# facebookresearch/pytorchvideo

Hardware: AMD Instinct MI355X
Metric: clips/sec forward (higher is better)
Workload: dtype bf16; 1 GPU; x3d_m: create_x3d(input_clip_length=16,input_crop_size=224) [B,3,16,224,224]; per_gpu_batch=32, global_batch=32, parallelism=dp1 (batch-sharded, logits all_gather), head_collective=none (one rank: the logits stay where they are), hip_graph=True, streams=2

## Files before the change

pytorchvideo_amd/csrc/pv_pwdw.hip:

```cpp
#include "pv_common.h"

int pv_plane_variant(const pv_dwconv3d_desc& d);
int pv_plane_tiles(const pv_dwconv3d_desc& d, int nw);

namespace {

constexpr int kPlaneThreads = 256;
constexpr int kPR = kPlaneThreads / 64;

template <int S, int NW, int KS, int ACT>
__global__ __launch_bounds__(kPlaneThreads) void pwdw_plane_kernel(const pv_dwconv3d_desc d, int ntiles, int ngroups) {
  constexpr int TW = 4 * NW;
  constexpr int IH = (kPR - 1) * S + 3;
  constexpr int IW = (TW - 1) * S + 3;
  constexpr bool kDeep = S == 1;
  constexpr int IWP = (IW + 1) & ~1;
  constexpr int NVOX = IH * IW;
  constexpr int NMT = (NVOX + 15) / 16;
  constexpr int MT = (NMT + kPR - 1) / kPR;
  constexpr int NC = (NW - 1) * S + 3;
  __shared__ __attribute__((aligned(16))) bf16_t s_in[2][IH * IWP + 1][32];
  __shared__ float s_ps[kPR][32];

  const int tid = threadIdx.x;
  const int lane = tid & 63;
  const int row = __builtin_amdgcn_readfirstlane(tid >> 6);
  const int cp = lane & 15;
  const int sx = lane >> 4;
  const int n16 = lane & 15, q = lane >> 4;
  const int c_p = pv_round_up(d.C, 8);
  const int xcd = blockIdx.x & 7, slot = blockIdx.x >> 3;
  const int grp = slot % ngroups;
  const long tb = (long)(slot / ngroups) * 8 + xcd;
  if (tb >= (long)ntiles * d.B) return;
  const int tile_id = (int)(tb % ntiles);
  const int cbase = grp * 32;
  const int ch = cbase + cp * 2;
  const bool ch_ok = ch < c_p;
  const int tiles_w = (d.Wo + TW - 1) / TW;
  const int th = tile_id / tiles_w, tw = tile_id - th * tiles_w;
  const int b = (int)(tb / ntiles);
  const int ho0 = th * kPR, wo0 = tw * TW;
  const int ho = ho0 + row, wo_first = wo0 + sx * NW;
  const int hi0 = ho0 * S - 1, wi0 = wo0 * S - 1;

  constexpr unsigned kOOB = 0x80000000u;
  const bf16_t* X = static_cast<const bf16_t*>(d.x) + (long)b * d.x_bs;
  bf16_t* Y = static_cast<bf16_t*>(d.y) + (long)b * d.y_bs;
  const unsigned x_plane_bytes = (unsigned)(d.Hi * d.Wi * d.ldx) * 2u;
  const unsigned y_plane_bytes = (unsigned)(d.Ho * d.Wo * d.ldy) * 2u;
  __amdgpu_buffer_rsrc_t rx = __builtin_amdgcn_make_buffer_rsrc((void*)X, 0, (int)(x_plane_bytes * (unsigned)d.Ti), 0x00020000);
  __amdgpu_buffer_rsrc_t ry = __builtin_amdgcn_make_buffer_rsrc((void*)Y, 0, (int)(y_plane_bytes * (unsigned)d.To), 0x00020000);

  float2 wt[27];
#pragma unroll
  for (int t = 0; t < 27; ++t)
    wt[t] = ch_ok ? *reinterpret_cast<const float2*>(d.w + (long)t * c_p + ch) : float2{0.f, 0.f};
  float2 sc = {0.f, 0.f}, sh = {0.f, 0.f};
  if (ch_ok) {
    sc.x = ch < d.C ? (d.scale ? d.scale[ch] : 1.f) : 0.f;
    sc.y = ch + 1 < d.C ? (d.scale ? d.scale[ch + 1] : 1.f) : 0.f;
    sh.x = ch < d.C ? (d.shift ? d.shift[ch] : 0.f) : 0.f;
    sh.y = ch + 1 < d.C ? (d.shift ? d.shift[ch + 1] : 0.f) : 0.f;
  }

  bf16x8 wa[2][KS];
  {
    const bf16_t* __restrict__ Wa = static_cast<const bf16_t*>(d.pw_w);
#pragma unroll
    for (int nt = 0; nt < 2; ++nt)
#pragma unroll
      for (int ks = 0; ks < KS; ++ks)
        wa[nt][ks] = *reinterpret_cast<const bf16x8*>(Wa + (long)(cbase + 8 * (n16 >> 2) + 4 * nt + (n16 & 3)) * (KS * 32) + ks * 32 + q * 8);
  }
  float2 sa[2][2], ha[2][2];
#pragma unroll
  for (int nt = 0; nt < 2; ++nt)
#pragma unroll
    for (int r = 0; r < 4; ++r) {
      const int c = cbase + q * 8 + nt * 4 + r;
      const bool ok = c < d.C;
      const float s_ = ok ? (d.pw_scale ? d.pw_scale[c] : 1.f) : 0.f;
      const float h_ = ok ? (d.pw_shift ? d.pw_shift[c] : 0.f) : 0.f;
      if (r & 1) { sa[nt][r >> 1].y = s_; ha[nt][r >> 1].y = h_; }
      else { sa[nt][r >> 1].x = s_; ha[nt][r >> 1].x = h_; }
    }
  const bool a_relu = d.pw_act == PV_ACT_RELU;

  auto colperm = [](int c) { return c ^ ((c / (NW * S)) & 1); };
  unsigned x_off[MT];
  int h_lds[MT];
#pragma unroll
  for (int i = 0; i < MT; ++i) {
    const int v = (row + i * kPR) * 16 + n16;
    const int ih = v / IW, iw = v - ih * IW;
    const int hi = hi0 + ih, wi = wi0 + iw;
    const bool in_tile = v < NVOX;
    const bool ok = in_tile && (unsigned)hi < (unsigned)d.Hi && (unsigned)wi < (unsigned)d.Wi;
    x_off[i] = ok ? (unsigned)((hi * d.Wi + wi) * d.ldx + q * 8) * 2u : kOOB;
    h_lds[i] = (in_tile ? ih * IWP + colperm(iw) : IH * IWP) * 32 + q * 8;
  }
  typedef unsigned int u32x4 __attribute__((ext_vector_type(4)));
  u32x4 xa[MT][KS], xb[MT][KS];
  auto load_plane = [&](u32x4 (&reg)[MT][KS], int p) {
    if (p >= d.Ti) return;
    const unsigned pb = (unsigned)p * x_plane_bytes;
#pragma unroll
    for (int i = 0; i < MT; ++i)
#pragma unroll
      for (int ks = 0; ks < KS; ++ks)
        reg[i][ks] = __builtin_amdgcn_raw_buffer_load_b128(rx, (int)(x_off[i] + pb + ks * 64u), 0, 0);
  };
  auto produce_plane = [&](const u32x4 (&reg)[MT][KS], int p) {
    if (p >= d.Ti) return;
    bf16_t* dst = &s_in[p & 1][0][0];
#pragma unroll
    for (int i = 0; i < MT; ++i) {
      f32x4 acc[2] = {f32x4{0.f, 0.f, 0.f, 0.f}, f32x4{0.f, 0.f, 0.f, 0.f}};
#pragma unroll
      for (int ks = 0; ks < KS; ++ks) {
        const bf16x8 xf = __builtin_bit_cast(bf16x8, reg[i][ks]);
        acc[0] = __builtin_amdgcn_mfma_f32_16x16x32_bf16(wa[0][ks], xf, acc[0], 0, 0, 0);
        acc[1] = __builtin_amdgcn_mfma_f32_16x16x32_bf16(wa[1][ks], xf, acc[1], 0, 0, 0);
      }
      const unsigned inside = x_off[i] != kOOB ? 0xffffffffu : 0u;
      u32x4 o;
#pragma unroll
      for (int nt = 0; nt < 2; ++nt) {
        typedef __bf16 bf16x2_t __attribute__((ext_vector_type(2)));
        typedef short s16x2 __attribute__((ext_vector_type(2)));
#pragma unroll
        for (int h = 0; h < 2; ++h) {
          const float v0 = acc[nt][2 * h] * sa[nt][h].x + ha[nt][h].x;
          const float v1 = acc[nt][2 * h + 1] * sa[nt][h].y + ha[nt][h].y;
          const bf16x2_t pk = {(bf16_t)v0, (bf16_t)v1};
          s16x2 pi = __builtin_bit_cast(s16x2, pk);
          if (a_relu) pi = __builtin_elementwise_max(pi, s16x2{0, 0});
          o[nt * 2 + h] = __builtin_bit_cast(unsigned, pi) & inside;
        }
      }
      *reinterpret_cast<u32x4*>(dst + h_lds[i]) = o;
    }
  };

  float2 acc[3][NW];
#pragma unroll
  for (int a = 0; a < 3; ++a)
#pragma unroll
    for (int n = 0; n < NW; ++n) acc[a][n] = float2{0.f, 0.f};
  float2 ps = {0.f, 0.f};

  unsigned y_off[NW];
  float y_mask[NW];
#pragma unroll
  for (int n = 0; n < NW; ++n) {
    const int wo = wo_first + n;
    const bool ok = ch_ok && ho < d.Ho && wo < d.Wo;
    y_off[n] = ok ? (unsigned)((ho * d.Wo + wo) * d.ldy + ch) * 2u : kOOB;
    y_mask[n] = ok ? 1.f : 0.f;
  }
  const bool has_psum = d.psum != nullptr;
  auto finalize = [&](float2 (&a)[NW], int t) {
    const unsigned tbytes = (unsigned)t * y_plane_bytes;
#pragma unroll
    for (int n = 0; n < NW; ++n) {
      float v0 = a[n].x * sc.x + sh.x, v1 = a[n].y * sc.y + sh.y;
      if (has_psum) { ps.x += v0 * y_mask[n]; ps.y += v1 * y_mask[n]; }
      if (ACT == PV_ACT_RELU) { v0 = fmaxf(v0, 0.f); v1 = fmaxf(v1, 0.f); }
      else if (ACT == PV_ACT_SWISH) { v0 *= pv_sigmoid(v0); v1 *= pv_sigmoid(v1); }
      typedef __bf16 bf16x2_t __attribute__((ext_vector_type(2)));
      const bf16x2_t o = {(bf16_t)v0, (bf16_t)v1};
      __builtin_amdgcn_raw_buffer_store_b32(__builtin_bit_cast(unsigned, o), ry, (int)(y_off[n] + tbytes), 0, 0);
    }
  };

  auto plane = [&](int p) {
    const bf16_t* base = &s_in[p & 1][0][0] + cp * 2;
#pragma unroll
    for (int dh = 0; dh < 3; ++dh) {
      float2 x[NC];
#pragma unroll
      for (int i = 0; i < NC; ++i) {
        const uint32_t u = *reinterpret_cast<const uint32_t*>(base + ((row * S + dh) * IWP + colperm(sx * NW * S + i)) * 32);
        x[i].x = __uint_as_float(u << 16);
        x[i].y = __uint_as_float(u & 0xffff0000u);
      }
#pragma unroll
      for (int dw = 0; dw < 3; ++dw) {
        const float2 w0 = wt[(0 * 3 + dh) * 3 + dw];
        const float2 w1 = wt[(1 * 3 + dh) * 3 + dw];
        const float2 w2 = wt[(2 * 3 + dh) * 3 + dw];
#pragma unroll
        for (int n = 0; n < NW; ++n) {
          const float2 xv = x[n * S + dw];
          acc[2][n].x += xv.x * w0.x; acc[2][n].y += xv.y * w0.y;
          acc[1][n].x += xv.x * w1.x; acc[1][n].y += xv.y * w1.y;
          acc[0][n].x += xv.x * w2.x; acc[0][n].y += xv.y * w2.y;
        }
      }
    }
    if (p >= 1) finalize(acc[0], p - 1);
    if (p == d.Ti - 1) finalize(acc[1], p);
#pragma unroll
    for (int n = 0; n < NW; ++n) {
      acc[0][n] = acc[1][n];
      acc[1][n] = acc[2][n];
      acc[2][n] = float2{0.f, 0.f};
    }
  };

  load_plane(xa, 0);
  if (kDeep) load_plane(xb, 1);
  produce_plane(xa, 0);
  __syncthreads();
  if (kDeep) {
    for (int p = 0; p < d.Ti; p += 2) {
      load_plane(xa, p + 2);
      plane(p);
      produce_plane(xb, p + 1);
      __syncthreads();
      if (p + 1 < d.Ti) {
        load_plane(xb, p + 3);
        plane(p + 1);
        produce_plane(xa, p + 2);
        __syncthreads();
      }
    }
  } else {
    for (int p = 0; p < d.Ti; ++p) {
      load_plane(xa, p + 1);
      plane(p);
      produce_plane(xa, p + 1);
      __syncthreads();
    }
  }

  if (d.psum != nullptr) {
    ps.x += __shfl_xor(ps.x, 16, 64); ps.y += __shfl_xor(ps.y, 16, 64);
    ps.x += __shfl_xor(ps.x, 32, 64); ps.y += __shfl_xor(ps.y, 32, 64);
    if (lane < 16) { s_ps[row][cp * 2] = ps.x; s_ps[row][cp * 2 + 1] = ps.y; }
    __syncthreads();
    if (tid < 32 && cbase + tid < c_p) {
      float a = 0.f;
#pragma unroll
      for (int rr = 0; rr < kPR; ++rr) a += s_ps[rr][tid];
      float* dst = d.psum + ((long)b * ntiles + tile_id) * c_p + cbase + tid;
      *dst = a;
    }
  }
}

template <int S, int NW, int KS> int launch_pwdw(const pv_dwconv3d_desc& d, hipStream_t s) {
  const int c_p = pv_round_up(d.C, 8);
  const int ntiles = pv_plane_tiles(d, NW), ngroups = (c_p + 31) / 32;
  const long blocks = pv_ceil_div((long)ntiles * d.B, 8) * 8 * ngroups;
  if (blocks > 0x7fffffffL) return PV_ERR_UNSUPPORTED;
  dim3 grid((unsigned)blocks), block(kPlaneThreads);
  if (d.act == PV_ACT_NONE) PV_LAUNCH((pwdw_plane_kernel<S, NW, KS, PV_ACT_NONE>), grid, block, 0, s, d, ntiles, ngroups);
  else if (d.act == PV_ACT_RELU) PV_LAUNCH((pwdw_plane_kernel<S, NW, KS, PV_ACT_RELU>), grid, block, 0, s, d, ntiles, ngroups);
  else PV_LAUNCH((pwdw_plane_kernel<S, NW, KS, PV_ACT_SWISH>), grid, block, 0, s, d, ntiles, ngroups);
  PV_LAUNCH_CHECK();
  return PV_OK;
}

template <int KS> int launch_ks(const pv_dwconv3d_desc& d, int nw, hipStream_t s) {
  if (d.sw == 1) return nw == 4 ? launch_pwdw<1, 4, KS>(d, s) : launch_pwdw<1, 2, KS>(d, s);
  return nw == 4 ? launch_pwdw<2, 4, KS>(d, s) : launch_pwdw<2, 2, KS>(d, s);
}

int ksteps_of(const pv_dwconv3d_desc& d) {
  const int ks = (d.pw_cin + 31) / 32;
  return (ks == 1 || ks == 2 || ks == 3 || ks == 4 || ks == 6) ? ks : 0;
}

}

int pv_pwdw_supported(const pv_dwconv3d_desc& d) {
  if (d.dtype != PV_BF16 || d.w_mod != 0 || d.n_prefix != 0) return 0;
  if (d.pw_cin <= 0 || d.ldx < pv_round_up(d.pw_cin, 8)) return 0;
  if (!ksteps_of(d)) return 0;
  if (d.pw_act != PV_ACT_NONE && d.pw_act != PV_ACT_RELU) return 0;
  return pv_plane_variant(d) != 0;
}

int pv_pwdw_launch(const pv_dwconv3d_desc& d, hipStream_t s) {
  if (!pv_pwdw_supported(d)) return PV_ERR_UNSUPPORTED;
  const int nw = pv_plane_variant(d);
  switch (ksteps_of(d)) {
    case 1: return launch_ks<1>(d, nw, s);
    case 2: return launch_ks<2>(d, nw, s);
    case 3: return launch_ks<3>(d, nw, s);
    case 4: return launch_ks<4>(d, nw, s);
    case 6: return launch_ks<6>(d, nw, s);
  }
  return PV_ERR_UNSUPPORTED;
}
```

Before: 11900 clips/s.

## Specialize pwdw plane kernel on relu/psum and software-pipeline pointwise MFMA epilogue

```diff
diff --git a/pytorchvideo_amd/csrc/pv_pwdw.hip b/pytorchvideo_amd/csrc/pv_pwdw.hip
--- a/pytorchvideo_amd/csrc/pv_pwdw.hip
+++ b/pytorchvideo_amd/csrc/pv_pwdw.hip
@@ -1,3 +1,5 @@
+#include <type_traits>
+
 #include "pv_common.h"
 
 int pv_plane_variant(const pv_dwconv3d_desc& d);
@@ -7,6 +9,19 @@
 
 constexpr int kPlaneThreads = 256;
 constexpr int kPR = kPlaneThreads / 64;
+
+__device__ __forceinline__ void mfma_first(f32x4& dst, const bf16x8& a, const bf16x8& b) {
+  asm volatile("v_mfma_f32_16x16x32_bf16 %0, %1, %2, 0" : "=&v"(dst) : "v"(a), "v"(b));
+}
+__device__ __forceinline__ void mfma_acc(f32x4& dst, const bf16x8& a, const bf16x8& b) {
+  asm volatile("v_mfma_f32_16x16x32_bf16 %0, %1, %2, %0" : "+v"(dst) : "v"(a), "v"(b));
+}
+__device__ __forceinline__ void mfma_wait(f32x4& c0, f32x4& c1) {
+  asm volatile("s_nop 7" : "+v"(c0), "+v"(c1));
+}
+template <typename V> __device__ __forceinline__ void mfma_after(f32x4& c0, f32x4& c1, const V& done) {
+  asm volatile("" : "+v"(c0), "+v"(c1) : "v"(done));
+}
 
 template <int S, int NW, int KS, int ACT>
 __global__ __launch_bounds__(kPlaneThreads) void pwdw_plane_kernel(const pv_dwconv3d_desc d, int ntiles, int ngroups) {
@@ -19,6 +34,8 @@
   constexpr int NMT = (NVOX + 15) / 16;
   constexpr int MT = (NMT + kPR - 1) / kPR;
   constexpr int NC = (NW - 1) * S + 3;
+  constexpr bool kTailStore = S == 1;
+  constexpr bool kArithMfma = KS <= 2;
   __shared__ __attribute__((aligned(16))) bf16_t s_in[2][IH * IWP + 1][32];
   __shared__ float s_ps[kPR][32];
 
@@ -52,10 +69,10 @@
   __amdgpu_buffer_rsrc_t rx = __builtin_amdgcn_make_buffer_rsrc((void*)X, 0, (int)(x_plane_bytes * (unsigned)d.Ti), 0x00020000);
   __amdgpu_buffer_rsrc_t ry = __builtin_amdgcn_make_buffer_rsrc((void*)Y, 0, (int)(y_plane_bytes * (unsigned)d.To), 0x00020000);
 
-  float2 wt[27];
+  f32x2 wt[27];
 #pragma unroll
   for (int t = 0; t < 27; ++t)
-    wt[t] = ch_ok ? *reinterpret_cast<const float2*>(d.w + (long)t * c_p + ch) : float2{0.f, 0.f};
+    wt[t] = ch_ok ? *reinterpret_cast<const f32x2*>(d.w + (long)t * c_p + ch) : f32x2{0.f, 0.f};
   float2 sc = {0.f, 0.f}, sh = {0.f, 0.f};
   if (ch_ok) {
     sc.x = ch < d.C ? (d.scale ? d.scale[ch] : 1.f) : 0.f;
@@ -85,9 +102,8 @@
       if (r & 1) { sa[nt][r >> 1].y = s_; ha[nt][r >> 1].y = h_; }
       else { sa[nt][r >> 1].x = s_; ha[nt][r >> 1].x = h_; }
     }
-  const bool a_relu = d.pw_act == PV_ACT_RELU;
-
   auto colperm = [](int c) { return c ^ ((c / (NW * S)) & 1); };
+  typedef unsigned int u32x4 __attribute__((ext_vector_type(4)));
   unsigned x_off[MT];
   int h_lds[MT];
 #pragma unroll
@@ -98,9 +114,13 @@
     const bool in_tile = v < NVOX;
     const bool ok = in_tile && (unsigned)hi < (unsigned)d.Hi && (unsigned)wi < (unsigned)d.Wi;
     x_off[i] = ok ? (unsigned)((hi * d.Wi + wi) * d.ldx + q * 8) * 2u : kOOB;
-    h_lds[i] = (in_tile ? ih * IWP + colperm(iw) : IH * IWP) * 32 + q * 8;
-  }
-  typedef unsigned int u32x4 __attribute__((ext_vector_type(4)));
+    h_lds[i] = (ok ? ih * IWP + colperm(iw) : IH * IWP) * 32 + q * 8;
+    if (in_tile && !ok) {
+      const int z = (ih * IWP + colperm(iw)) * 32 + q * 8;
+      *reinterpret_cast<u32x4*>(&s_in[0][0][0] + z) = u32x4{0u, 0u, 0u, 0u};
+      *reinterpret_cast<u32x4*>(&s_in[1][0][0] + z) = u32x4{0u, 0u, 0u, 0u};
+    }
+  }
   u32x4 xa[MT][KS], xb[MT][KS];
   auto load_plane = [&](u32x4 (&reg)[MT][KS], int p) {
     if (p >= d.Ti) return;
@@ -109,46 +129,30 @@
     for (int i = 0; i < MT; ++i)
 #pragma unroll
       for (int ks = 0; ks < KS; ++ks)
-        reg[i][ks] = __builtin_amdgcn_raw_buffer_load_b128(rx, (int)(x_off[i] + pb + ks * 64u), 0, 0);
+        reg[i][ks] = __builtin_amdgcn_raw_buffer_load_b128(rx, (int)(x_off[i] + ks * 64u), (int)pb, 0);
   };
-  auto produce_plane = [&](const u32x4 (&reg)[MT][KS], int p) {
-    if (p >= d.Ti) return;
-    bf16_t* dst = &s_in[p & 1][0][0];
-#pragma unroll
-    for (int i = 0; i < MT; ++i) {
-      f32x4 acc[2] = {f32x4{0.f, 0.f, 0.f, 0.f}, f32x4{0.f, 0.f, 0.f, 0.f}};
-#pragma unroll
-      for (int ks = 0; ks < KS; ++ks) {
-        const bf16x8 xf = __builtin_bit_cast(bf16x8, reg[i][ks]);
-        acc[0] = __builtin_amdgcn_mfma_f32_16x16x32_bf16(wa[0][ks], xf, acc[0], 0, 0, 0);
-        acc[1] = __builtin_amdgcn_mfma_f32_16x16x32_bf16(wa[1][ks], xf, acc[1], 0, 0, 0);
-      }
-      const unsigned inside = x_off[i] != kOOB ? 0xffffffffu : 0u;
-      u32x4 o;
-#pragma unroll
-      for (int nt = 0; nt < 2; ++nt) {
-        typedef __bf16 bf16x2_t __attribute__((ext_vector_type(2)));
-        typedef short s16x2 __attribute__((ext_vector_type(2)));
-#pragma unroll
-        for (int h = 0; h < 2; ++h) {
-          const float v0 = acc[nt][2 * h] * sa[nt][h].x + ha[nt][h].x;
-          const float v1 = acc[nt][2 * h + 1] * sa[nt][h].y + ha[nt][h].y;
-          const bf16x2_t pk = {(bf16_t)v0, (bf16_t)v1};
-          s16x2 pi = __builtin_bit_cast(s16x2, pk);
-          if (a_relu) pi = __builtin_elementwise_max(pi, s16x2{0, 0});
-          o[nt * 2 + h] = __builtin_bit_cast(unsigned, pi) & inside;
-        }
-      }
-      *reinterpret_cast<u32x4*>(dst + h_lds[i]) = o;
+  auto conv_a = [&](f32x4 (&c)[2], const u32x4 (&reg)[KS]) {
+#pragma unroll
+    for (int ks = 0; ks < KS; ++ks) {
+      const bf16x8 xf = __builtin_bit_cast(bf16x8, reg[ks]);
+      if constexpr (!kArithMfma) {
+        c[0] = __builtin_amdgcn_mfma_f32_16x16x32_bf16(wa[0][ks], xf, ks ? c[0] : f32x4{0.f, 0.f, 0.f, 0.f}, 0, 0, 0);
+        c[1] = __builtin_amdgcn_mfma_f32_16x16x32_bf16(wa[1][ks], xf, ks ? c[1] : f32x4{0.f, 0.f, 0.f, 0.f}, 0, 0, 0);
+      } else if (ks == 0) {
+        mfma_first(c[0], wa[0][ks], xf);
+        mfma_first(c[1], wa[1][ks], xf);
+      } else {
+        mfma_acc(c[0], wa[0][ks], xf);
+        mfma_acc(c[1], wa[1][ks], xf);
+      }
     }
   };
-
-  float2 acc[3][NW];
+  f32x2 acc[3][NW];
 #pragma unroll
   for (int a = 0; a < 3; ++a)
 #pragma unroll
-    for (int n = 0; n < NW; ++n) acc[a][n] = float2{0.f, 0.f};
-  float2 ps = {0.f, 0.f};
+    for (int n = 0; n < NW; ++n) acc[a][n] = f32x2{0.f, 0.f};
+  f32x2 ps = {0.f, 0.f};
 
   unsigned y_off[NW];
   float y_mask[NW];
@@ -159,80 +163,148 @@
     y_off[n] = ok ? (unsigned)((ho * d.Wo + wo) * d.ldy + ch) * 2u : kOOB;
     y_mask[n] = ok ? 1.f : 0.f;
   }
-  const bool has_psum = d.psum != nullptr;
-  auto finalize = [&](float2 (&a)[NW], int t) {
+  static_assert(NW * S % 2 == 0 && NC <= 2 * NW * S, "column groups of the pair swap");
+  int col[2][2];
+#pragma unroll
+  for (int g = 0; g < 2; ++g)
+#pragma unroll
+    for (int par = 0; par < 2; ++par) {
+      const int t = (sx + g) & 1;
+      col[g][par] = ((row * S * IWP + sx * NW * S + (par ? -t : t)) * 32 + cp * 2) * 2;
+      asm volatile("" : "+v"(col[g][par]));
+    }
+
+  auto finalize = [&](f32x2 (&a)[NW], int t, auto sums_c) {
     const unsigned tbytes = (unsigned)t * y_plane_bytes;
 #pragma unroll
     for (int n = 0; n < NW; ++n) {
       float v0 = a[n].x * sc.x + sh.x, v1 = a[n].y * sc.y + sh.y;
-      if (has_psum) { ps.x += v0 * y_mask[n]; ps.y += v1 * y_mask[n]; }
+      if (decltype(sums_c)::value) {
+        ps = __builtin_elementwise_fma(f32x2{v0, v1}, f32x2{y_mask[n], y_mask[n]}, ps);
+      }
       if (ACT == PV_ACT_RELU) { v0 = fmaxf(v0, 0.f); v1 = fmaxf(v1, 0.f); }
       else if (ACT == PV_ACT_SWISH) { v0 *= pv_sigmoid(v0); v1 *= pv_sigmoid(v1); }
       typedef __bf16 bf16x2_t __attribute__((ext_vector_type(2)));
       const bf16x2_t o = {(bf16_t)v0, (bf16_t)v1};
-      __builtin_amdgcn_raw_buffer_store_b32(__builtin_bit_cast(unsigned, o), ry, (int)(y_off[n] + tbytes), 0, 0);
+      __builtin_amdgcn_raw_buffer_store_b32(__builtin_bit_cast(unsigned, o), ry, (int)y_off[n], (int)tbytes, 0);
     }
   };
 
-  auto plane = [&](int p) {
-    const bf16_t* base = &s_in[p & 1][0][0] + cp * 2;
-#pragma unroll
-    for (int dh = 0; dh < 3; ++dh) {
-      float2 x[NC];
-#pragma unroll
-      for (int i = 0; i < NC; ++i) {
-        const uint32_t u = *reinterpret_cast<const uint32_t*>(base + ((row * S + dh) * IWP + colperm(sx * NW * S + i)) * 32);
-        x[i].x = __uint_as_float(u << 16);
-        x[i].y = __uint_as_float(u & 0xffff0000u);
-      }
-#pragma unroll
-      for (int dw = 0; dw < 3; ++dw) {
-        const float2 w0 = wt[(0 * 3 + dh) * 3 + dw];
-        const float2 w1 = wt[(1 * 3 + dh) * 3 + dw];
-        const float2 w2 = wt[(2 * 3 + dh) * 3 + dw];
-#pragma unroll
-        for (int n = 0; n < NW; ++n) {
-          const float2 xv = x[n * S + dw];
-          acc[2][n].x += xv.x * w0.x; acc[2][n].y += xv.y * w0.y;
-          acc[1][n].x += xv.x * w1.x; acc[1][n].y += xv.y * w1.y;
-          acc[0][n].x += xv.x * w2.x; acc[0][n].y += xv.y * w2.y;
-        }
-      }
-    }
-    if (p >= 1) finalize(acc[0], p - 1);
-    if (p == d.Ti - 1) finalize(acc[1], p);
-#pragma unroll
-    for (int n = 0; n < NW; ++n) {
-      acc[0][n] = acc[1][n];
-      acc[1][n] = acc[2][n];
-      acc[2][n] = float2{0.f, 0.f};
+  auto walk = [&](auto relu_c, auto psum_c) {
+    constexpr bool a_relu = decltype(relu_c)::value;
+    auto produce_plane = [&](const u32x4 (&reg)[MT][KS], int p) {
+      if (p >= d.Ti) return;
+      bf16_t* dst = &s_in[p & 1][0][0];
+      f32x4 c[2][2];
+      u32x4 o;
+      conv_a(c[0], reg[0]);
+#pragma unroll
+      for (int i = 0; i < MT; ++i) {
+        f32x4 (&ci)[2] = c[i & 1];
+        if (i + 1 < MT) conv_a(c[(i + 1) & 1], reg[i + 1]);
+        if (kArithMfma && i == 0) mfma_wait(ci[0], ci[1]);
+        else if (kArithMfma) mfma_after(ci[0], ci[1], o);
+#pragma unroll
+        for (int nt = 0; nt < 2; ++nt) {
+          typedef __bf16 bf16x2_t __attribute__((ext_vector_type(2)));
+          typedef short s16x2 __attribute__((ext_vector_type(2)));
+#pragma unroll
+          for (int h = 0; h < 2; ++h) {
+            const float v0 = ci[nt][2 * h] * sa[nt][h].x + ha[nt][h].x;
+            const float v1 = ci[nt][2 * h + 1] * sa[nt][h].y + ha[nt][h].y;
+            const bf16x2_t pk = {(bf16_t)v0, (bf16_t)v1};
+            s16x2 pi = __builtin_bit_cast(s16x2, pk);
+            if (a_relu) pi = __builtin_elementwise_max(pi, s16x2{0, 0});
+            o[nt * 2 + h] = __builtin_bit_cast(unsigned, pi);
+          }
+        }
+        *reinterpret_cast<u32x4*>(dst + h_lds[i]) = o;
+      }
+    };
+
+    auto plane = [&](int p) {
+      const char* base = reinterpret_cast<const char*>(&s_in[p & 1][0][0]);
+#pragma unroll
+      for (int dh = 0; dh < 3; ++dh) {
+        f32x2 x[NC];
+#pragma unroll
+        for (int i = 0; i < NC; ++i) {
+          const uint32_t u = *reinterpret_cast<const uint32_t*>(base + col[i / (NW * S)][i & 1] + (dh * IWP + i) * 64);
+          x[i].x = __uint_as_float(u << 16);
+          x[i].y = __uint_as_float(u & 0xffff0000u);
+        }
+#pragma unroll
+        for (int dw = 0; dw < 3; ++dw) {
+          const f32x2 w0 = wt[(0 * 3 + dh) * 3 + dw];
+          const f32x2 w1 = wt[(1 * 3 + dh) * 3 + dw];
+          const f32x2 w2 = wt[(2 * 3 + dh) * 3 + dw];
+#pragma unroll
+          for (int n = 0; n < NW; ++n) {
+            const f32x2 xv = x[n * S + dw];
+            if constexpr (S == 2 && NW == 4) {
+              if (n == 1) {
+#pragma clang fp contract(off)
+                acc[2][n] = acc[2][n] + xv * w0;
+              } else {
+                acc[2][n] = __builtin_elementwise_fma(xv, w0, acc[2][n]);
+              }
+            } else {
+              acc[2][n] = __builtin_elementwise_fma(xv, w0, acc[2][n]);
+            }
+            acc[1][n] = __builtin_elementwise_fma(xv, w1, acc[1][n]);
+            acc[0][n] = __builtin_elementwise_fma(xv, w2, acc[0][n]);
+          }
+        }
+      }
+      if (p >= 1) finalize(acc[0], p - 1, psum_c);
+      if (!kTailStore && p == d.Ti - 1) finalize(acc[1], p, psum_c);
+#pragma unroll
+      for (int n = 0; n < NW; ++n) {
+        acc[0][n] = acc[1][n];
+        acc[1][n] = acc[2][n];
+        acc[2][n] = f32x2{0.f, 0.f};
+      }
+    };
+
+    load_plane(xa, 0);
+    if (kDeep) load_plane(xb, 1);
+    produce_plane(xa, 0);
+    __syncthreads();
+    if (kDeep) {
+      for (int p = 0; p < d.Ti; p += 2) {
+        load_plane(xa, p + 2);
+        plane(p);
+        produce_plane(xb, p + 1);
+        __syncthreads();
+        if (p + 1 < d.Ti) {
+          load_plane(xb, p + 3);
+          plane(p + 1);
+          produce_plane(xa, p + 2);
+          __syncthreads();
+        }
+      }
+    } else {
+      for (int p = 0; p < d.Ti; p += 2) {
+        load_plane(xa, p + 1);
+        plane(p);
+        produce_plane(xa, p + 1);
+        __syncthreads();
+        if (p + 1 < d.Ti) {
+          load_plane(xa, p + 2);
+          plane(p + 1);
+          produce_plane(xa, p + 2);
+          __syncthreads();
+        }
+      }
     }
   };
-
-  load_plane(xa, 0);
-  if (kDeep) load_plane(xb, 1);
-  produce_plane(xa, 0);
-  __syncthreads();
-  if (kDeep) {
-    for (int p = 0; p < d.Ti; p += 2) {
-      load_plane(xa, p + 2);
-      plane(p);
-      produce_plane(xb, p + 1);
-      __syncthreads();
-      if (p + 1 < d.Ti) {
-        load_plane(xb, p + 3);
-        plane(p + 1);
-        produce_plane(xa, p + 2);
-        __syncthreads();
-      }
-    }
-  } else {
-    for (int p = 0; p < d.Ti; ++p) {
-      load_plane(xa, p + 1);
-      plane(p);
-      produce_plane(xa, p + 1);
-      __syncthreads();
-    }
+  {
+    using yes = std::true_type;
+    using no = std::false_type;
+    const bool relu = d.pw_act == PV_ACT_RELU, sums = d.psum != nullptr;
+    if (relu) { if (sums) walk(yes{}, yes{}); else walk(yes{}, no{}); }
+    else { if (sums) walk(no{}, yes{}); else walk(no{}, no{}); }
+    if (kTailStore && d.Ti > 0) { if (sums) finalize(acc[0], d.Ti - 1, yes{}); else finalize(acc[0], d.Ti - 1, no{}); }
   }
 
   if (d.psum != nullptr) {
```

Measured after the change: 12140 clips/s (median of 6 runs). 2.0% higher.
